# axlwild/dna-kmeres-parallel

Measured on AMD Instinct MI355X. Metric: k-mers/sec (whole node), 10 Gbase synthetic FASTA, at 1/2/4/8 MI355X, higher is better.
Workload: dtype u8

## Files before the change

dna-kmeres-parallel_amd/csrc/kmc_dense.hip:

```cpp
#include <hip/hip_runtime.h>

#include <algorithm>
#include <atomic>
#include <cstdint>
#include <cstdio>
#include <cstdlib>
#include <mutex>
#include <vector>

#include "kmc.h"
#include "kmc_internal.h"
#include "kmc_stream.h"
#include "kmc_workspace.h"

namespace kmc {
constexpr int kHm3Scan = 256;
constexpr int kChunk = 16;
thread_local hipEvent_t t_trace_before = nullptr;
thread_local hipEvent_t t_trace_after = nullptr;
namespace {

struct Spill {
    int64_t rec;
    int32_t code;
    int32_t amount;
};

struct Params {
    const char *data;
    const void *indices;
    int64_t ibias;
    int64_t n;
    int32_t *sum;
    int64_t ld;
    int32_t *invalid;
    int64_t wl, wh, rl, rh;
    int derive;
    int G;
    uint32_t *slab;
    int64_t *slot_rec;
    Spill *spill;
    uint32_t *spill_cnt;
    uint32_t spill_cap;
    uint32_t *status;
};

__device__ __forceinline__ void raise_status(uint32_t *st, uint32_t code) {
    if (st) __hip_atomic_store(st, code, __ATOMIC_RELAXED, __HIP_MEMORY_SCOPE_SYSTEM);
}

__device__ __forceinline__ uint32_t half_inc(uint32_t hb) {
    uint32_t r;
    asm("v_mad_u32_u24 %0, %1, %2, 1" : "=v"(r) : "v"(hb), "s"(0xFFFFu));
    return r;
}

struct P16Ctx {
    uint32_t *h;
    uint32_t *spilled;
    uint32_t *spill_n;
    Spill *spill;
    uint32_t cap;
    int64_t rec;
};

__device__ __forceinline__ void p16_spill(const P16Ctx &c, int32_t code, int32_t amount) {
    const uint32_t i = atomicAdd(c.spill_n, 1u);
    if (i < c.cap) {
        Spill e;
        e.rec = c.rec;
        e.code = code;
        e.amount = amount;
        c.spill[i] = e;
    }
}

__device__ __noinline__ void p16_fix(const P16Ctx &c, uint32_t word, uint32_t hb, uint32_t hiwrap) {
    if (hb == 0u) {
        p16_spill(c, (int32_t)word, 65536);
        if (hiwrap) p16_spill(c, (int32_t)(word | 0x8000u), 65536);
        const uint32_t o2 = __hip_atomic_fetch_add(&c.h[word], 0xFFFF0000u, __ATOMIC_RELAXED,
                                                   __HIP_MEMORY_SCOPE_WORKGROUP);
        if ((o2 >> 16) == 0u) p16_spill(c, (int32_t)(word | 0x8000u), -65536);
    } else {
        p16_spill(c, (int32_t)(word | 0x8000u), 65536);
    }
}

template <int K, int J>
__device__ __forceinline__ uint32_t window_code(uint32_t lo, uint32_t mid) {
    constexpr uint32_t M = (K == 16) ? 0xFFFFFFFFu : ((1u << (2 * K)) - 1u);
    if constexpr (J <= 16 - K)
        return (lo >> (2 * J)) & M;
    else
        return (mid >> (2 * (J - 8))) & M;
}

template <int K, int R, int J, bool MASKED>
__device__ __forceinline__ void add32(uint32_t lo, uint32_t mid, uint32_t W, uint32_t *h, uint32_t rep) {
    const uint32_t code = window_code<K, J>(lo, mid);
    if (!MASKED || ((W >> J) & 1u))
        __hip_atomic_fetch_add(&h[code * R + rep], 1u, __ATOMIC_RELAXED, __HIP_MEMORY_SCOPE_WORKGROUP);
}

template <int K, int R, bool MASKED>
__device__ __forceinline__ void count_tile32(uint32_t lo, uint32_t hi, uint32_t W, uint32_t *h, int lane) {
    const uint32_t mid = __builtin_amdgcn_alignbit(hi, lo, 16);
    const uint32_t rep = (uint32_t)(lane & (R - 1));
    add32<K, R, 0, MASKED>(lo, mid, W, h, rep);
    add32<K, R, 1, MASKED>(lo, mid, W, h, rep);
    add32<K, R, 2, MASKED>(lo, mid, W, h, rep);
    add32<K, R, 3, MASKED>(lo, mid, W, h, rep);
    add32<K, R, 4, MASKED>(lo, mid, W, h, rep);
    add32<K, R, 5, MASKED>(lo, mid, W, h, rep);
    add32<K, R, 6, MASKED>(lo, mid, W, h, rep);
    add32<K, R, 7, MASKED>(lo, mid, W, h, rep);
    add32<K, R, 8, MASKED>(lo, mid, W, h, rep);
    add32<K, R, 9, MASKED>(lo, mid, W, h, rep);
    add32<K, R, 10, MASKED>(lo, mid, W, h, rep);
    add32<K, R, 11, MASKED>(lo, mid, W, h, rep);
    add32<K, R, 12, MASKED>(lo, mid, W, h, rep);
    add32<K, R, 13, MASKED>(lo, mid, W, h, rep);
    add32<K, R, 14, MASKED>(lo, mid, W, h, rep);
    add32<K, R, 15, MASKED>(lo, mid, W, h, rep);
}

template <bool MASKED>
__device__ __forceinline__ void count_tile_p16_plain(uint32_t lo, uint32_t hi, uint32_t W, uint32_t *h) {
// ... 35 lines not shown
        w[q] = (lo & (T - 1)) | ((hi & (T - 1)) << 16);
    }
}

template <int BLOCK, uint32_t T>
__device__ __forceinline__ void p16_scan(const P16Ctx &pc) {
    constexpr uint32_t HOT = (0xFFFFu & ~(T - 1)) * 0x00010001u;
    constexpr int NW4 = (1 << 15) / 4;
    const uint4 *h4 = reinterpret_cast<const uint4 *>(pc.h);
    uint32_t hot = 0u;
#pragma unroll
    for (int i = 0; i < NW4 / BLOCK; ++i) {
        const uint4 v = h4[threadIdx.x + i * BLOCK];
        hot |= (uint32_t)(((v.x | v.y | v.z | v.w) & HOT) != 0u) << i;
    }
    if (hot) {
        for (int i = 0; i < NW4 / BLOCK; ++i)
            if ((hot >> i) & 1u) p16_scan_fix<T>(pc, (int)threadIdx.x + i * BLOCK);
    }
}

template <int K, int R, int HM, int BLOCK>
struct DenseOp {
    static_assert(HM == 0 || HM == 3, "histogram modes: 0 (32-bit bins) and 3 (k = 8 packed halves)");
    uint32_t *h;
    int lane;
    const P16Ctx &pc;
    uint32_t nwin = 0u;

    __device__ DenseOp(uint32_t *h_, int lane_, const P16Ctx &pc_) : h(h_), lane(lane_), pc(pc_) {}

    __device__ __forceinline__ void before_tile() {}
    template <bool MASKED>
    __device__ __forceinline__ void tile(uint32_t lo, uint32_t hi, uint32_t W) {
        count_tile<K, R, HM, MASKED>(lo, hi, W, h, lane);
        if constexpr (HM == 3) nwin += MASKED ? (uint32_t)__builtin_popcount(W) : 16u;
    }
    __device__ __forceinline__ void segment_end() {
        if constexpr (HM == 3) {
            lds_barrier();
            p16_scan<BLOCK, 32768u>(pc);
            lds_barrier();
        }
    }
    static constexpr int kSegChunks = HM == 3 ? BLOCK / 64 * kHm3Scan / kChunk : 0;
    __device__ __forceinline__ void after_iter(int64_t, int64_t, bool) {}
};

template <int BLOCK>
__device__ __noinline__ void recount_p16(const char *data, int64_t ps, int64_t pe, int64_t rl, int64_t rh,
                                         const P16Ctx &pc) {
    constexpr int K = 8;
    const int64_t per = (pe - ps + BLOCK - 1) / BLOCK;
    const int64_t i0 = ps + (int64_t)threadIdx.x * per;
    const int64_t i1 = (i0 + per) < pe ? (i0 + per) : pe;
    uint32_t code = 0u, run = 0u;
    for (int64_t b = i0; b < i1 + K - 1; ++b) {
        const uint32_t c = (b >= rl && b < rh) ? (uint32_t)(uint8_t)data[b] : 0u;
        const uint32_t v = c == 'A' ? 0u : c == 'C' ? 1u : c == 'G' ? 2u : c == 'T' ? 3u : 4u;
        run = v < 4u ? run + 1u : 0u;
        code = (code >> 2) | ((v & 3u) << (2 * K - 2));
        if (run >= (uint32_t)K) {
            const uint32_t word = code & 0x7FFFu, hb = code >> 15;
            const uint32_t old = __hip_atomic_fetch_add(&pc.h[word], half_inc(hb), __ATOMIC_RELAXED,
                                                        __HIP_MEMORY_SCOPE_WORKGROUP);
            const uint32_t m = hb ? 0xFFFF0000u : 0x0000FFFFu;
            if ((old & m) == m) p16_fix(pc, word, hb, old >= 0xFFFF0000u ? 1u : 0u);
        }
    }
}

template <int K, int R, int HM, class Idx, int BLOCK>
__global__ __launch_bounds__(BLOCK) void count_dense_kernel(Params p) {
    constexpr bool P16 = HM != 0;
    constexpr int NB = 1 << (2 * K);
    constexpr int NW = P16 ? NB / 2 : NB * R;
    __shared__ __attribute__((aligned(16))) uint32_t smem[NW + 8];
    uint32_t *h = smem;
    uint32_t *misc = smem + NW;

    const int tid = threadIdx.x, lane = tid & 63;
    const int w = blockIdx.x;
    const Geom g = make_geom<Idx>(p);
    const int64_t tb = g.T0 + (int64_t)w * g.tpw;
    const int64_t te = (tb + g.tpw) < g.T1 ? (tb + g.tpw) : g.T1;
    int64_t slot0 = -1, slot1 = -1;

    if (tb < te) {
        const int64_t R0 = (tb << kTileShift) > g.wl ? (tb << kTileShift) : g.wl;
        const int64_t R1 = (te << kTileShift) < g.wh ? (te << kTileShift) : g.wh;
        int64_t s0 = 0;
        if (p.n <= BLOCK) {
            if (tid == 0) {
                misc[0] = 0u;
                misc[3] = 0u;
                misc[4] = 0u;
                misc[5] = 0u;
                misc[7] = 0u;
            }
            const bool le = tid < p.n && rec_off<Idx>(p, tid) <= R0;
            for (int i = tid; i < NW / 4; i += BLOCK) reinterpret_cast<uint4 *>(h)[i] = make_uint4(0u, 0u, 0u, 0u);
            const int cnt = __syncthreads_count(le);
            s0 = cnt > 0 ? cnt - 1 : 0;
        } else {
            if (tid == 0) {
                int64_t lo = 0, hi = p.n - 1;
                if (rec_off<Idx>(p, 0) <= R0) {
                    while (lo < hi) {
                        const int64_t mid = (lo + hi + 1) >> 1;
                        if (rec_off<Idx>(p, mid) <= R0) lo = mid;
                        else hi = mid - 1;
                    }
                }
                misc[0] = 0u;
                misc[3] = 0u;
                misc[4] = 0u;
                misc[5] = 0u;
                misc[7] = 0u;
                misc[1] = (uint32_t)lo;
                misc[2] = (uint32_t)((uint64_t)lo >> 32);
            }
            for (int i = tid; i < NW / 4; i += BLOCK) reinterpret_cast<uint4 *>(h)[i] = make_uint4(0u, 0u, 0u, 0u);
            __syncthreads();
            s0 = (int64_t)((uint64_t)misc[1] | ((uint64_t)misc[2] << 32));
        }

        P16Ctx pc;
        pc.h = h;
        pc.spilled = misc + 5;
        pc.spill_n = misc;
        pc.spill = p.spill ? p.spill + (int64_t)w * p.spill_cap : nullptr;
        pc.cap = p.spill_cap;

        int npieces = 0;
        for (int64_t s = s0; s < p.n; ++s) {
            if (rec_off<Idx>(p, s) >= R1) break;
            int64_t ca, ce;
            record_windows<K, Idx>(p, g, s, ca, ce);
            const int64_t ps = ca > R0 ? ca : R0;
            const int64_t pe = ce < R1 ? ce : R1;
            if (ps >= pe) continue;
            pc.rec = s;
            const int64_t tp0 = ps >> kTileShift;
            const int64_t tp1 = ((pe - 1) >> kTileShift) + 1;
            using Op = DenseOp<K, R, HM, BLOCK>;
            Op op(h, lane, pc);
            if constexpr (K >= 7) {
                stream_chunks<K, kChunk, Op::kSegChunks>(p.data, tp0, tp1, ps, pe, g.rl, g.rh, lane, &misc[7], op);
            } else {
                constexpr int NWAVES = BLOCK / 64;
                const int wave = __builtin_amdgcn_readfirstlane(tid >> 6);
                const int64_t per = (tp1 - tp0 + NWAVES - 1) / NWAVES;
                const int64_t a0 = tp0 + (int64_t)wave * per;
                const int64_t a1 = (a0 + per) < tp1 ? (a0 + per) : tp1;
                stream_tiles<K>(p.data, a0, a1, per, ps, pe, g.rl, g.rh, lane, op);
            }
            if constexpr (HM == 3) {
                const uint32_t wsum = wave_sum(op.nwin);
                if (lane == 0) atomicAdd(&misc[3], wsum);
            }
            __syncthreads();
            const bool entire = (ps == ca) && (pe == ce);
            int slot = 0;
            if (!entire) {
                slot = (npieces == 0) ? 0 : 1;
                if (slot == 0) slot0 = s;
                else slot1 = s;
            }
            uint32_t *dst = p.slab + ((int64_t)w * 2 + slot) * NB;
            if constexpr (P16) {
                const auto flush = [&]() {
                    uint32_t dsum = 0u;
                    if (!entire) {
                        for (int i = tid; i < NW / 4; i += BLOCK) {
                            const uint4 v = reinterpret_cast<const uint4 *>(h)[i];
                            reinterpret_cast<uint4 *>(h)[i] = make_uint4(0u, 0u, 0u, 0u);
                            dsum += (v.x & 0xFFFFu) + (v.x >> 16) + (v.y & 0xFFFFu) + (v.y >> 16) + (v.z & 0xFFFFu) +
                                    (v.z >> 16) + (v.w & 0xFFFFu) + (v.w >> 16);
                            reinterpret_cast<uint4 *>(dst)[i] = v;
                        }
                        return dsum;
                    }
                    for (int i = tid; i < NW; i += BLOCK) {
                        const uint32_t v = h[i];
                        h[i] = 0u;
                        dsum += (v & 0xFFFFu) + (v >> 16);
                        if (entire) {
                            p.sum[s + p.ld * (int64_t)i] = (int32_t)(v & 0xFFFFu);
                            p.sum[s + p.ld * (int64_t)(i + NW)] = (int32_t)(v >> 16);
                        } else {
                            dst[i] = v;
                        }
                    }
                    return dsum;
                };
                const uint32_t dsum = flush();
                if constexpr (HM == 3) {
                    const uint32_t wsum = wave_sum(dsum);
                    if (lane == 0) atomicAdd(&misc[4], wsum);
                    __syncthreads();
                    if (tid == 0) {
                        misc[6] = misc[3] != misc[4] + misc[5] ? 1u : 0u;
                        misc[3] = 0u;
                        misc[4] = 0u;
                        misc[5] = 0u;
                    }
                    __syncthreads();
                    if (misc[6]) {
                        const uint32_t n0 = misc[0] < pc.cap ? misc[0] : pc.cap;
                        for (uint32_t i = tid; i < n0; i += BLOCK)
                            if (pc.spill[i].rec == s) pc.spill[i].amount = 0;
                        __syncthreads();
                        recount_p16<BLOCK>(p.data, ps, pe, g.rl, g.rh, pc);
                        __syncthreads();
                        (void)flush();
                    }
                }
            } else {
                for (int c = tid; c < NB; c += BLOCK) {
                    uint32_t v = 0;
#pragma unroll
                    for (int r = 0; r < R; ++r) {
                        v += h[c * R + r];
                        h[c * R + r] = 0u;
                    }
                    if (entire) p.sum[s + p.ld * (int64_t)c] = (int32_t)v;
                    else dst[c] = v;
                }
            }
            if (tid == 0) misc[7] = 0u;
            __syncthreads();
            ++npieces;
        }
    }
    if (tid == 0) {
        p.slot_rec[2 * w] = slot0;
        p.slot_rec[2 * w + 1] = slot1;
        if (p.spill_cnt) {
            p.spill_cnt[w] = (tb < te) ? misc[0] : 0u;
            if (tb < te && misc[0] > p.spill_cap) raise_status(p.status, KMC_ERR_CAPACITY);
        }
    }
}

template <int K, class Idx, bool P16>
__global__ __launch_bounds__(256) void reduce_dense_kernel(Params p) {
    constexpr int NB = 1 << (2 * K);
    constexpr int NW = P16 ? NB / 2 : NB;
    constexpr int RC = NW / 4 < 16 ? NW / 4 : 16;
    constexpr int RR = 256 / RC;
    constexpr int RW = 4 * RC;
    constexpr int NH = P16 ? 2 : 1;
    __shared__ uint32_t s_part[RR][RW * NH];
    __shared__ uint32_t s_out[RW * NH];
    const int tid = threadIdx.x, col = tid % RC, row = tid / RC;
    const int64_t c0 = (int64_t)blockIdx.x * RW;
    const Geom g = make_geom<Idx>(p);
    const auto for_spills = [&](int64_t s, int64_t wf, int64_t wlast, auto &&f) {
        for (int64_t l = wf; l <= wlast; ++l) {
            const uint32_t c = p.spill_cnt[l] < p.spill_cap ? p.spill_cnt[l] : p.spill_cap;
            const Spill *sp = p.spill + l * (int64_t)p.spill_cap;
            uint32_t lo = 0u, hi = c;
            while (lo < hi) {
                const uint32_t mid = (lo + hi) >> 1;
                if (sp[mid].rec < s) lo = mid + 1u;
                else hi = mid;
            }
            for (uint32_t i = lo + tid; i < c; i += 256) {
                const Spill e = sp[i];
                if (e.rec != s) break;
                const int64_t wd = (int64_t)(e.code & (NW - 1)) - c0;
                if (e.amount != 0 && wd >= 0 && wd < RW) f((int)wd + (e.code / NW) * RW, e.amount);
            }
        }
    };
    for (int64_t s = blockIdx.y; s < p.n; s += gridDim.y) {
        int64_t ca, ce;
        record_windows<K, Idx>(p, g, s, ca, ce);
        if (blockIdx.x == 0 && tid == 0 && ce - ca >= ((int64_t)1 << 31)) raise_status(p.status, KMC_ERR_RECORD_TOO_LONG);
        if (ce <= ca) {
            for (int i = tid; i < RW * NH; i += 256) {
                const int64_t c = c0 + i % RW + (i / RW) * NW;
                p.sum[s + p.ld * c] = 0;
            }
            continue;
        }
        const int64_t wf = ((ca >> kTileShift) - g.T0) / g.tpw;
        const int64_t wlast = (((ce - 1) >> kTileShift) - g.T0) / g.tpw;
        bool spills = false;
        if constexpr (P16) {
            uint32_t any = 0u;
            for (int64_t l = wf + tid; l <= wlast; l += 256) any |= p.spill_cnt[l];
            spills = __syncthreads_or(any != 0u) != 0;
        }
        if (wf == wlast) {
            if (spills)
                for_spills(s, wf, wlast, [&](int i, int32_t a) {
                    atomicAdd(&p.sum[s + p.ld * (c0 + i % RW + (i / RW) * (int64_t)NW)], a);
                });
            continue;
        }
        uint32_t acc[4 * NH] = {};
        const int64_t sf = 2 * wf + (p.slot_rec[2 * wf] == s ? 0 : 1);
        const int64_t n = wlast - wf + 1;
#pragma unroll 4
        for (int64_t i = row; i < n; i += RR) {
            const int64_t slot = i == 0 ? sf : 2 * (wf + i);
            const uint4 v = reinterpret_cast<const uint4 *>(p.slab + slot * NB + c0)[col];
            const uint32_t x[4] = {v.x, v.y, v.z, v.w};
#pragma unroll
            for (int e = 0; e < 4; ++e) {
                if constexpr (P16) {
                    acc[e] += x[e] & 0xFFFFu;
                    acc[4 + e] += x[e] >> 16;
                } else {
                    acc[e] += x[e];
                }
            }
        }
#pragma unroll
        for (int e = 0; e < 4 * NH; ++e) s_part[row][(e / 4) * RW + col * 4 + e % 4] = acc[e];
        __syncthreads();
        for (int i = tid; i < RW * NH; i += 256) {
            uint32_t t = 0u;
#pragma unroll 8
            for (int r = 0; r < RR; ++r) t += s_part[r][i];
            s_out[i] = t;
        }
        if (spills) {
            __syncthreads();
            for_spills(s, wf, wlast, [&](int i, int32_t a) { atomicAdd(&s_out[i], (uint32_t)a); });
        }
        __syncthreads();
        for (int i = tid; i < RW * NH; i += 256) {
            const int64_t c = c0 + i % RW + (i / RW) * NW;
            p.sum[s + p.ld * c] = (int32_t)s_out[i];
        }
        __syncthreads();
    }
}


template <int K, class Idx>
__global__ __launch_bounds__(256) void invalid_kernel(Params p) {
    constexpr int NB = 1 << (2 * K);
    __shared__ int64_t red[256];
    for (int64_t s = blockIdx.x; s < p.n; s += gridDim.x) {
        int64_t acc = 0;
        for (int c = threadIdx.x; c < NB; c += 256) acc += p.sum[s + p.ld * (int64_t)c];
        red[threadIdx.x] = acc;
        __syncthreads();
        for (int st = 128; st > 0; st >>= 1) {
            if ((int)threadIdx.x < st) red[threadIdx.x] += red[threadIdx.x + st];
            __syncthreads();
        }
        if (threadIdx.x == 0) {
            const Geom g = make_geom<Idx>(p);
            int64_t ca, ce;
            record_windows<K, Idx>(p, g, s, ca, ce);
            const int64_t nw = ce > ca ? ce - ca : 0;
            p.invalid[s] = (int32_t)(nw - red[0]);
        }
        __syncthreads();
    }
}

template <int K>
struct Cfg;
template <> struct Cfg<1> { static constexpr int R = 32, BLOCK = 512, HM = 0; static constexpr bool P16 = false; };
template <> struct Cfg<2> { static constexpr int R = 32, BLOCK = 512, HM = 0; static constexpr bool P16 = false; };
template <> struct Cfg<3> { static constexpr int R = 32, BLOCK = 512, HM = 0; static constexpr bool P16 = false; };
template <> struct Cfg<4> { static constexpr int R = 32, BLOCK = 512, HM = 0; static constexpr bool P16 = false; };
template <> struct Cfg<5> { static constexpr int R = 8, BLOCK = 512, HM = 0; static constexpr bool P16 = false; };
template <> struct Cfg<6> { static constexpr int R = 2, BLOCK = 512, HM = 0; static constexpr bool P16 = false; };
template <> struct Cfg<7> { static constexpr int R = 1, BLOCK = 512, HM = 0; static constexpr bool P16 = false; };
template <> struct Cfg<8> { static constexpr int R = 1, BLOCK = 1024, HM = 3; static constexpr bool P16 = true; };

struct DevInfo {
    int occ[KMC_DENSE_MAX_K + 1][2] = {};
    uint32_t *status_host = nullptr;
    uint32_t *status_dev = nullptr;
};

std::mutex g_mu;
std::vector<DevInfo> g_dev;


template <int K, class Idx>
void *kernel_ptr() {
    return reinterpret_cast<void *>(&count_dense_kernel<K, Cfg<K>::R, Cfg<K>::HM, Idx, Cfg<K>::BLOCK>);
}

thread_local int t_reserved_cus = 0;

#ifdef KMC_DIAG_HOOKS
std::atomic<uint32_t> g_diag_spill_cap{0};
#endif

template <int K, class Idx>
int grid_size(int device, int &G) {
    int dev_cus = 0;
    if (int e = device_cus(device, &dev_cus)) return e;
    std::lock_guard<std::mutex> lk(g_mu);
    if ((int)g_dev.size() <= device) g_dev.resize(device + 1);
    DevInfo &d = g_dev[device];
    const int ix = sizeof(Idx) == 8 ? 1 : 0;
    if (d.occ[K][ix] == 0) {
        const void *kp = kernel_ptr<K, Idx>();
        int nb = 0;
        hipError_t e = hipOccupancyMaxActiveBlocksPerMultiprocessor(&nb, kp, Cfg<K>::BLOCK, 0);
        if (e != hipSuccess) return (int)e;
        d.occ[K][ix] = nb > 0 ? nb : 1;
    }
    const int cus = dev_cus - t_reserved_cus;
    G = (cus > 0 ? cus : 1) * d.occ[K][ix];
    return 0;
}

int status_flag(int device, uint32_t **host, uint32_t **dev) {
    std::lock_guard<std::mutex> lk(g_mu);
    if ((int)g_dev.size() <= device) g_dev.resize(device + 1);
    DevInfo &d = g_dev[device];
    if (!d.status_host) {
        void *h = nullptr;
        hipError_t e = hipHostMalloc(&h, sizeof(uint32_t), hipHostMallocMapped | hipHostMallocCoherent);
        if (e != hipSuccess) return KMC_ERR_NOMEM;
        void *dp = nullptr;
        e = hipHostGetDevicePointer(&dp, h, 0);
        if (e != hipSuccess) {
            (void)hipHostFree(h);
            return (int)e;
        }
        *static_cast<volatile uint32_t *>(h) = 0u;
        d.status_host = static_cast<uint32_t *>(h);
        d.status_dev = static_cast<uint32_t *>(dp);
    }
    *host = d.status_host;
    *dev = d.status_dev;
    return 0;
}

int take_status(int device) {
    uint32_t *h = nullptr;
    {
        std::lock_guard<std::mutex> lk(g_mu);
        if ((int)g_dev.size() > device && device >= 0) h = g_dev[device].status_host;
    }
    if (!h) return KMC_OK;
    const uint32_t v = __atomic_exchange_n(h, 0u, __ATOMIC_ACQ_REL);
    return (int)v;
}

struct WsLayout {
    int64_t *slot_rec;
    uint32_t *spill_cnt, *slab;
    Spill *spill;
    size_t total;
};

inline WsLayout ws_layout(void *base, int k, int G, uint32_t spill_cap) {
    const size_t nb = (size_t)1 << (2 * k);
    Carver c(base);
    WsLayout L;
    L.slot_rec = c.take<int64_t>((size_t)G * 2);
    L.spill_cnt = c.take<uint32_t>((size_t)G);
    L.slab = c.take<uint32_t>((size_t)G * 2 * nb);
    L.spill = c.take<Spill>((size_t)G * spill_cap);
    L.total = c.total();
    return L;
}

constexpr uint32_t kSpillWindowsPerEntry = 4096;
static_assert(5u * kSpillWindowsPerEntry <= 65536u, "HM 3 scan + HM 1 recount entries exceed the spill cap");
inline uint32_t spill_cap_for(int64_t tiles_per_wg) {
    const int64_t windows = tiles_per_wg * kTile;
    return (uint32_t)(windows / kSpillWindowsPerEntry + 64);
}

struct Plan {
    int G;
    uint32_t spill_cap;
    size_t ws_bytes;
};

template <int K, class Idx>
int make_plan(int device, bool derive, int64_t wl, int64_t wh, Plan &pl) {
    int G = 0;
    int e = grid_size<K, Idx>(device, G);
    if (e) return e;
    pl.spill_cap = 0;
    if (!derive) {
        const int64_t tiles = wh > wl ? ((wh + kTile - 1) >> kTileShift) - (wl >> kTileShift) : 0;
        if (tiles < G) G = tiles > 0 ? (int)tiles : 1;
        const int64_t tpw = tiles > 0 ? (tiles + G - 1) / G : 1;
        if (Cfg<K>::P16) {
            pl.spill_cap = spill_cap_for(tpw);
#ifdef KMC_DIAG_HOOKS
            const uint32_t dc = g_diag_spill_cap.load();
            if (dc) pl.spill_cap = dc;
#endif
        }
    }
    pl.G = G;
    pl.ws_bytes = ws_layout(nullptr, K, G, pl.spill_cap).total;
    return 0;
}

DeviceCache g_ws;

struct Request {
    const char *data;
    const void *indices;
    int64_t ibias;
    int64_t n;
    int32_t *sum;
    int64_t ld;
    int32_t *invalid;
    bool derive;
    int64_t wl, wh, rl, rh;
    void *ws;
    size_t ws_bytes;
    uint32_t *status;
};

template <int K, class Idx>
int run_dense(const Request &q, hipStream_t st) {
    int device = 0;
    hipError_t he = hipGetDevice(&device);
    if (he != hipSuccess) return (int)he;
    bool derive = q.derive;
    int64_t wl = q.wl, wh = q.wh, rl = q.rl, rh = q.rh;
    if (derive && Cfg<K>::P16) {
        Idx ends[2];
        he = hipMemcpyAsync(&ends[0], q.indices, sizeof(Idx), hipMemcpyDeviceToHost, st);
        if (he == hipSuccess)
            he = hipMemcpyAsync(&ends[1], (const Idx *)q.indices + q.n, sizeof(Idx), hipMemcpyDeviceToHost, st);
        if (he == hipSuccess) he = hipStreamSynchronize(st);
        if (he != hipSuccess) return (int)he;
        wl = rl = (int64_t)ends[0] + q.ibias;
        wh = rh = (int64_t)ends[1] + q.ibias;
        derive = false;
    }
    Plan pl;
    int e = make_plan<K, Idx>(device, derive, wl, wh, pl);
    if (e) return e;
    void *ws = nullptr;
    if ((e = bind_workspace(g_ws, device, pl.ws_bytes, q.ws, q.ws_bytes, 0, &ws))) return e;
    const WsLayout L = ws_layout(ws, K, pl.G, pl.spill_cap);
    Params p;
    p.data = q.data;
    p.indices = q.indices;
    p.ibias = q.ibias;
    p.n = q.n;
    p.sum = q.sum;
    p.ld = q.ld;
    p.invalid = q.invalid;
    p.wl = wl;
    p.wh = wh;
    p.rl = rl;
    p.rh = rh;
    p.derive = derive ? 1 : 0;
    p.G = pl.G;
    p.slot_rec = L.slot_rec;
    p.spill_cnt = Cfg<K>::P16 ? L.spill_cnt : nullptr;
    p.slab = L.slab;
    p.spill = Cfg<K>::P16 ? L.spill : nullptr;
    p.spill_cap = pl.spill_cap;
    p.status = q.status;
    if (!p.status) {
        uint32_t *sh = nullptr;
        e = status_flag(device, &sh, &p.status);
        if (e) return e;
    }

    constexpr int NB = 1 << (2 * K);
    if (t_trace_before) {
        he = hipEventRecord(t_trace_before, st);
        if (he != hipSuccess) return (int)he;
    }
    hipLaunchKernelGGL((count_dense_kernel<K, Cfg<K>::R, Cfg<K>::HM, Idx, Cfg<K>::BLOCK>), dim3(pl.G),
                       dim3(Cfg<K>::BLOCK), 0, st, p);
    he = hipGetLastError();
    if (he != hipSuccess) return (int)he;
    if (t_trace_after) {
        he = hipEventRecord(t_trace_after, st);
        if (he != hipSuccess) return (int)he;
    }
    constexpr int NWR = Cfg<K>::P16 ? NB / 2 : NB;
    constexpr int RW = NWR / 4 < 16 ? NWR : 64;
    const unsigned cb = (unsigned)(NWR / RW);
    hipLaunchKernelGGL((reduce_dense_kernel<K, Idx, Cfg<K>::P16>), dim3(cb, (unsigned)std::min<int64_t>(q.n, kMaxGridY)),
                       dim3(256), 0, st, p);
    he = hipGetLastError();
    if (he != hipSuccess) return (int)he;
    if (q.invalid) {
        hipLaunchKernelGGL((invalid_kernel<K, Idx>), dim3((unsigned)std::min<int64_t>(q.n, kMaxGridX)), dim3(256), 0,
                           st, p);
        he = hipGetLastError();
        if (he != hipSuccess) return (int)he;
    }
    return 0;
}

template <class Idx>
int dispatch(int k, const Request &q, hipStream_t st) {
    switch (k) {
        case 1: return run_dense<1, Idx>(q, st);
        case 2: return run_dense<2, Idx>(q, st);
        case 3: return run_dense<3, Idx>(q, st);
        case 4: return run_dense<4, Idx>(q, st);
        case 5: return run_dense<5, Idx>(q, st);
        case 6: return run_dense<6, Idx>(q, st);
        case 7: return run_dense<7, Idx>(q, st);
        case 8: return run_dense<8, Idx>(q, st);
        default: return KMC_ERR_UNSUPPORTED_K;
    }
}

template <class Idx>
size_t workspace_for(int k, int device, bool derive, int64_t wl, int64_t wh) {
    Plan pl;
    int e = 0;
    switch (k) {
        case 1: e = make_plan<1, Idx>(device, derive, wl, wh, pl); break;
        case 2: e = make_plan<2, Idx>(device, derive, wl, wh, pl); break;
        case 3: e = make_plan<3, Idx>(device, derive, wl, wh, pl); break;
        case 4: e = make_plan<4, Idx>(device, derive, wl, wh, pl); break;
        case 5: e = make_plan<5, Idx>(device, derive, wl, wh, pl); break;
        case 6: e = make_plan<6, Idx>(device, derive, wl, wh, pl); break;
        case 7: e = make_plan<7, Idx>(device, derive, wl, wh, pl); break;
        case 8: e = make_plan<8, Idx>(device, derive, wl, wh, pl); break;
        default: return 0;
    }
    return e ? 0 : pl.ws_bytes;
}

}
}

using namespace kmc;

extern "C" int kmc_set_reserved_cus(int n) {
    if (n < 0 || n > 64) return KMC_ERR_INVALID_ARG;
    t_reserved_cus = n;
    return KMC_OK;
}

extern "C" int kmc_dense_status(int device) { return take_status(device); }

#ifdef KMC_DIAG_HOOKS
extern "C" KMC_DIAG_API int kmc_diag_dense_spill_cap(unsigned cap) {
    g_diag_spill_cap.store(cap);
    return KMC_OK;
}
#endif

extern "C" int kmc_trace_set_events(hipEvent_t before, hipEvent_t after) {
    t_trace_before = before;
    t_trace_after = after;
    return KMC_OK;
}

extern "C" int sumKmereCoincidencesGlobalMemory_hip(char *data, int *indices, unsigned num_seqs, int *sum,
                                                    hipStream_t stream) {
    if (num_seqs == 0) return KMC_OK;
    if (!data || !indices || !sum) return KMC_ERR_INVALID_ARG;
    const uintptr_t mis = reinterpret_cast<uintptr_t>(data) & 15u;
    Request q{};
    q.data = data - mis;
    q.ibias = (int64_t)mis;
    q.indices = indices;
    q.n = num_seqs;
    q.sum = sum;
// ... 103 lines not shown
```

dna-kmeres-parallel_amd/csrc/kmc_stream.h:

```cpp
#pragma once

#include <hip/hip_runtime.h>

#include <cstdint>

namespace kmc {

constexpr int kStreamPF = 3;
constexpr int kStreamNT = 1;

constexpr int kTileShift = 10;
constexpr int kTile = 1 << kTileShift;

constexpr uint32_t kCodeLo = 0x01000000u;
constexpr uint32_t kCodeHi = 0x02000003u;
constexpr uint32_t kCanonLo = 0x43FF41FFu;
constexpr uint32_t kCanonHi = 0x47FFFF54u;

__device__ __forceinline__ uint32_t byte_codes(uint32_t w) {
    return __builtin_amdgcn_perm(kCodeHi, kCodeLo, w & 0x07070707u);
}
__device__ __forceinline__ uint32_t byte_mismatch(uint32_t w) {
    return w ^ __builtin_amdgcn_perm(kCanonHi, kCanonLo, w & 0x07070707u);
}
// ... 42 lines not shown
}

template <int K>
__device__ __forceinline__ uint32_t smear(uint32_t x) {
    uint32_t s = x;
    int c = 1;
#pragma unroll
    for (int it = 0; it < 6; ++it) {
        if (c < K) {
            const int st = (c < K - c) ? c : (K - c);
            s |= s >> st;
            c += st;
        }
    }
    return s;
}

__device__ __forceinline__ uint32_t from_next_lane(uint32_t x) {
    return (uint32_t)__builtin_amdgcn_update_dpp(0, (int)x, 0x130, 0xF, 0xF, false);
}

__device__ __forceinline__ uint32_t wave_incl_scan(uint32_t x) {
    x += (uint32_t)__builtin_amdgcn_update_dpp(0, (int)x, 0x111, 0xF, 0xF, true);
    x += (uint32_t)__builtin_amdgcn_update_dpp(0, (int)x, 0x112, 0xF, 0xF, true);
    x += (uint32_t)__builtin_amdgcn_update_dpp(0, (int)x, 0x114, 0xF, 0xF, true);
    x += (uint32_t)__builtin_amdgcn_update_dpp(0, (int)x, 0x118, 0xF, 0xF, true);
    x += (uint32_t)__builtin_amdgcn_update_dpp(0, (int)x, 0x142, 0xA, 0xF, false);
    x += (uint32_t)__builtin_amdgcn_update_dpp(0, (int)x, 0x143, 0xC, 0xF, false);
    return x;
}

__device__ __forceinline__ uint32_t wave_sum(uint32_t x) {
#pragma unroll
    for (int o = 32; o > 0; o >>= 1) x += __shfl_xor(x, o);
    return x;
}

__device__ __forceinline__ void quad_bcast4(uint32_t x, uint32_t *o) {
    o[0] = (uint32_t)__builtin_amdgcn_update_dpp(0, (int)x, 0x00, 0xF, 0xF, false);
    o[1] = (uint32_t)__builtin_amdgcn_update_dpp(0, (int)x, 0x55, 0xF, 0xF, false);
    o[2] = (uint32_t)__builtin_amdgcn_update_dpp(0, (int)x, 0xAA, 0xF, 0xF, false);
    o[3] = (uint32_t)__builtin_amdgcn_update_dpp(0, (int)x, 0xFF, 0xF, 0xF, false);
}

__device__ __forceinline__ void lds_barrier() {
    __builtin_amdgcn_fence(__ATOMIC_RELEASE, "workgroup", "local");
    __builtin_amdgcn_s_barrier();
    __builtin_amdgcn_fence(__ATOMIC_ACQUIRE, "workgroup", "local");
}

struct Geom {
    int64_t wl, wh, rl, rh;
    int64_t T0, T1, tpw;
};

template <class Idx, class P>
__device__ __forceinline__ int64_t rec_off(const P &p, int64_t i) {
    return (int64_t)((const Idx *)p.indices)[i] + p.ibias;
}

template <class Idx, class P>
__device__ __forceinline__ Geom make_geom(const P &p) {
    Geom g;
    if (p.derive) {
        g.wl = rec_off<Idx>(p, 0);
        g.wh = rec_off<Idx>(p, p.n);
        g.rl = g.wl;
        g.rh = g.wh;
    } else {
        g.wl = p.wl;
        g.wh = p.wh;
        g.rl = p.rl;
        g.rh = p.rh;
    }
    if (g.wh <= g.wl) {
        g.T0 = g.T1 = 0;
        g.tpw = 1;
    } else {
        g.T0 = g.wl >> kTileShift;
        g.T1 = (g.wh + kTile - 1) >> kTileShift;
        g.tpw = (g.T1 - g.T0 + p.G - 1) / p.G;
    }
    return g;
}

template <int K, class Idx, class P>
__device__ __forceinline__ void record_windows(const P &p, const Geom &g, int64_t s, int64_t &ca,
                                               int64_t &ce) {
    const int64_t a = rec_off<Idx>(p, s);
    const int64_t e = rec_off<Idx>(p, s + 1);
    const int64_t nw = e - a - K > 0 ? e - a - K : 0;
    ca = a > g.wl ? a : g.wl;
    ce = (a + nw) < g.wh ? (a + nw) : g.wh;
}


template <class Idx, class P>
__device__ __forceinline__ int64_t first_record_at(const P &p, int64_t pos) {
    int64_t lo = 0, hi = p.n - 1;
    if (rec_off<Idx>(p, 0) <= pos) {
        while (lo < hi) {
            const int64_t mid = (lo + hi + 1) >> 1;
            if (rec_off<Idx>(p, mid) <= pos) lo = mid;
            else hi = mid - 1;
        }
    }
    return lo;
}

__device__ __forceinline__ __amdgpu_buffer_rsrc_t tile_rsrc(const char *data, int64_t base_off, int64_t rh) {
    const int64_t rh16 = (rh + 15) & ~(int64_t)15;
    int64_t nrec = rh16 - base_off;
    nrec = nrec < 0 ? 0 : (nrec > (1ll << 31) ? (1ll << 31) : nrec);
    return __builtin_amdgcn_make_buffer_rsrc(const_cast<char *>(data) + base_off, (short)0, (int)nrec,
                                             0x00020000);
}

__device__ __forceinline__ int64_t tile_base(int64_t t, int64_t rl) {
    const int64_t b = t << kTileShift, rl16 = rl & ~(int64_t)15;
    return b > rl16 ? b : rl16;
}

template <int NT = kStreamNT>
__device__ __forceinline__ uint4 load_tile_fast(__amdgpu_buffer_rsrc_t rsrc, int64_t base_off, int64_t t,
                                                int lane) {
    const int64_t off = (t << kTileShift) - base_off + (int64_t)lane * 16;
    typedef unsigned u32x4 __attribute__((ext_vector_type(4)));
    const u32x4 x = __builtin_amdgcn_raw_buffer_load_b128(rsrc, (int)(uint32_t)off, 0, NT ? 2 : 0);
    return make_uint4(x[0], x[1], x[2], x[3]);
}

__device__ __forceinline__ bool tile_straddles(int64_t t, int64_t rl, int64_t rh) {
    const int64_t b = t << kTileShift;
    return ((rl & 15) != 0 && rl > b && rl < b + kTile) || ((rh & 15) != 0 && rh > b && rh < b + kTile);
}

__device__ __forceinline__ uint4 mask_range(uint4 v, int64_t q, int64_t rl, int64_t rh) {
    const int64_t lo = rl - q, hi = rh - q;
    uint32_t w[4] = {v.x, v.y, v.z, v.w};
#pragma unroll
    for (int d = 0; d < 4; ++d) {
        int64_t a = lo - 4 * d, b = hi - 4 * d;
        a = a < 0 ? 0 : (a > 4 ? 4 : a);
        b = b < 0 ? 0 : (b > 4 ? 4 : b);
        uint32_t m = 0u;
        if (b > a) {
            const uint32_t upto = b == 4 ? 0xFFFFFFFFu : ((1u << (8 * (uint32_t)b)) - 1u);
            m = upto & ~((1u << (8 * (uint32_t)a)) - 1u);
        }
        w[d] &= m;
    }
    return make_uint4(w[0], w[1], w[2], w[3]);
}

template <int K, int PF_ = kStreamPF, int NT_ = kStreamNT>
struct TileStream {
    static constexpr int PF = PF_;
    static constexpr int NT = NT_;
    static constexpr int NS = PF + 1;
    const char *__restrict__ data;
    int64_t t0, ps, pe, rl, rh;
    int lane;
    __amdgpu_buffer_rsrc_t rsrc;
    int64_t base_off;
    uint4 r[NS];
    uint32_t c_cur, v_cur;
// ... 226 lines not shown
```

dna-kmeres-parallel_amd/kmc.py:

```python
import ctypes
import os
import re

import numpy as np

HERE = os.path.dirname(os.path.abspath(__file__))
REPO = os.path.dirname(HERE)
LIB_PATH = os.environ.get("KMC_LIB") or os.path.join(HERE, "lib", "libkmc.so")
DIAG_LIB_PATH = os.environ.get("KMC_DIAG_LIB") or os.path.join(HERE, "lib", "libkmc_diag.so")
HEADER = os.path.join(REPO, "include", "kmc.h")

DIALECT_BLANK = 0
DIALECT_NONL = 1
MAX_SEQS_REFERENCE = 100
DROPIN_K = 3
KMC_ERR_CAPACITY = 1009
KMC_ERR_RECORD_TOO_LONG = 1010
KMC_ERR_INTERNAL = 1011


class KmcError(RuntimeError):
    def __init__(self, code, what):
        self.code = code
        super().__init__("%s failed: %s (%d)" % (what, error_string(code), code))


_P = ctypes.c_void_p
_U64 = ctypes.c_uint64
_I64 = ctypes.c_int64


class DenseArgs(ctypes.Structure):
    _fields_ = [
        ("data", _P), ("indices", _P), ("num_seqs", _U64), ("k", ctypes.c_int),
        ("sum", _P), ("sum_ld", _U64), ("invalid", _P),
        ("read_lo", _U64), ("read_hi", _U64), ("win_lo", _U64), ("win_hi", _U64),
        ("workspace", _P), ("workspace_bytes", ctypes.c_size_t), ("status", _P),
    ]


_lib = None
_diag_lib = None
_active = None


def lib():
    global _lib
    if _active is not None:
        return _active
    if _lib is None:
        _lib = _load(LIB_PATH)
    return _lib


class diag:

    def __enter__(self):
        global _diag_lib, _active
        if _diag_lib is None:
            _diag_lib = _load(DIAG_LIB_PATH)
            _diag_lib.kmc_diag_radix_mode.argtypes = [ctypes.c_int, ctypes.c_float]
            _diag_lib.kmc_diag_canon_claim_cap.argtypes = [ctypes.c_uint]
            _diag_lib.kmc_diag_canon_sort_cap.argtypes = [ctypes.c_uint]
            _diag_lib.kmc_diag_canon_sort_cap_big.argtypes = [ctypes.c_uint]
            _diag_lib.kmc_diag_canon_direct.argtypes = [ctypes.c_int]
            _diag_lib.kmc_diag_canon_fallback.argtypes = [ctypes.POINTER(ctypes.c_ulonglong)] * 2
            _diag_lib.kmc_diag_canon_fallback_detail.argtypes = [ctypes.POINTER(ctypes.c_ulonglong), ctypes.c_uint,
                                                                 ctypes.POINTER(ctypes.c_ulonglong)]
            _diag_lib.kmc_diag_dense_spill_cap.argtypes = [ctypes.c_uint]
            _diag_lib.kmc_diag_canon_stale_queue.argtypes = [ctypes.c_longlong]
        self._prev = _active
        _active = _diag_lib
        return _diag_lib

    def __exit__(self, *exc):
        global _active
        L = _active
        L.kmc_diag_radix_mode(0, 1.0)
        L.kmc_diag_canon_claim_cap(0)
        L.kmc_diag_canon_sort_cap(1 << 30)
        L.kmc_diag_canon_direct(1)
        L.kmc_diag_dense_spill_cap(0)
        L.kmc_diag_canon_stale_queue(-1)
        _active = self._prev
        return False


def hip_runtimes():
    with open("/proc/self/maps") as f:
        return sorted(set(line.split()[-1] for line in f if "/libamdhip64.so" in line))


def _load(path):
    if not os.path.exists(path):
        raise RuntimeError("%s not built: run `make -C %s` (no CPU fallback exists)" % (os.path.basename(path), HERE))
    if os.environ.get("KMC_NO_TORCH") != "1":
        try:
            import torch
        except ImportError:
            pass
    L = ctypes.CDLL(path)
    rt = hip_runtimes()
    if len(rt) > 1:
        raise RuntimeError("two HIP runtimes are mapped in this process (%s): each would initialise the GPU on its "
                           "own, so %s is refused; import torch before loading it (or set KMC_NO_TORCH=1 only in "
                           "processes that never import torch)" % (", ".join(rt), os.path.basename(path)))
    L.kmc_error_string.restype = ctypes.c_char_p
    L.kmc_error_string.argtypes = [ctypes.c_int]
    L.kmc_version.restype = ctypes.c_int
    L.kmc_version.argtypes = []
    L.sumKmereCoincidencesGlobalMemory_hip.argtypes = [_P, _P, ctypes.c_uint, _P, _P]
    L.kmc_count_dense_workspace_size.restype = ctypes.c_size_t
    L.kmc_count_dense_workspace_size.argtypes = [ctypes.c_int, _U64, _U64, ctypes.c_int]
    L.kmc_count_dense.argtypes = [_P, _P, _U64, _U64, ctypes.c_int, _P, _P, _P, ctypes.c_size_t, _P]
    L.kmc_count_dense_ex.argtypes = [ctypes.POINTER(DenseArgs), _P]
    L.kmc_count_dense_ex_workspace_size.restype = ctypes.c_size_t
    L.kmc_count_dense_ex_workspace_size.argtypes = [ctypes.POINTER(DenseArgs), ctypes.c_int]
    L.kmc_dense_status.argtypes = [ctypes.c_int]
    L.kmc_trace_set_events.argtypes = [_P, _P]
    L.kmc_set_reserved_cus.argtypes = [ctypes.c_int]
    L.kmc_plan_shards.argtypes = [_P, _U64, ctypes.c_int, ctypes.c_int, _U64, _P]
    L.kmc_count_multi.argtypes = [_P, _P, _U64, _U64, ctypes.c_int, ctypes.c_int, _P, _P, _P]
    L.kmc_multi_release.argtypes = []
    L.kmc_synth_fill.argtypes = [_P, _U64, _U64, _U64, _U64, _P]
    L.kmc_synth_fill_range.argtypes = [_P, _U64, _U64, _U64, _U64, _P]
    L.kmc_synth_indices.argtypes = [_P, _U64, _U64]
    L.kmc_synth_indices.restype = None
    L.kmc_fasta_load.argtypes = [ctypes.c_char_p, ctypes.c_int, _I64, ctypes.POINTER(_P)]
    for fn in ("kmc_fasta_num_seqs", "kmc_fasta_data_bytes", "kmc_fasta_reference_num_indexes"):
        getattr(L, fn).restype = _U64
        getattr(L, fn).argtypes = [_P]
    L.kmc_fasta_indices.restype = _P
    L.kmc_fasta_indices.argtypes = [_P]
    L.kmc_fasta_data.restype = _P
    L.kmc_fasta_data.argtypes = [_P]
    L.kmc_fasta_free.argtypes = [_P]
    L.kmc_fasta_free.restype = None
    L.kmc_fasta_parse_device.argtypes = [_P, _U64, ctypes.c_int, _P, _U64, _P, _U64, ctypes.POINTER(_U64),
                                         ctypes.POINTER(_U64), _P]
    L.kmc_fasta_load_device.argtypes = [ctypes.c_char_p, ctypes.c_int, _I64, ctypes.POINTER(_P),
                                        ctypes.POINTER(_U64), ctypes.POINTER(_P), ctypes.POINTER(_U64), _P]
    L.kmc_pair_distances_workspace_size.restype = ctypes.c_size_t
    L.kmc_pair_distances_workspace_size.argtypes = [_U64, ctypes.c_int, ctypes.c_int]
    L.kmc_pair_distances.argtypes = [_P, _U64, _P, _U64, ctypes.c_int, _P, _P, ctypes.c_size_t, _P]
    L.kmc_pair_distances_sparse_workspace_size.restype = ctypes.c_size_t
    L.kmc_pair_distances_sparse_workspace_size.argtypes = [_U64, _U64, ctypes.c_int]
    L.kmc_pair_distances_sparse.argtypes = [_P, _P, _P, _U64, _P, _U64, ctypes.c_int, _P, _P, ctypes.c_size_t, _P]
    L.kmc_sketch_workspace_size.restype = ctypes.c_size_t
    L.kmc_sketch_workspace_size.argtypes = [_U64, _U64, ctypes.c_uint32, ctypes.c_int]
    L.kmc_sketch_from_counts.argtypes = [_P, _P, _P, _U64, _U64, ctypes.c_uint32, _U64, ctypes.c_uint32, _P, _P, _P,
                                         ctypes.c_size_t, _P]
    L.kmc_sketch_distances.argtypes = [_P, _P, _U64, ctypes.c_uint32, ctypes.c_int, _P, _P, _P, _P]
    L.kmc_sketch_from_sequences_workspace_size.restype = ctypes.c_size_t
    L.kmc_sketch_from_sequences_workspace_size.argtypes = [_U64, _U64, ctypes.c_uint32, ctypes.c_int]
    L.kmc_sketch_from_sequences.argtypes = [_P, _P, _U64, _U64, ctypes.c_int, ctypes.c_uint, ctypes.c_uint32, _U64,
                                            _P, _P, _P, ctypes.c_size_t, _P]
    L.kmc_sketch_from_sequences_grouped_workspace_size.restype = ctypes.c_size_t
    L.kmc_sketch_from_sequences_grouped_workspace_size.argtypes = [_U64, _U64, _U64, ctypes.c_uint32, ctypes.c_int]
    L.kmc_sketch_from_sequences_grouped.argtypes = [_P, _P, _U64, _U64, _P, _U64, ctypes.c_int, ctypes.c_uint,
                                                    ctypes.c_uint32, _U64, _P, _P, _P, ctypes.c_size_t, _P]
    L.kmc_sketch_merge_groups.argtypes = [_P, _P, _U64, _P, _U64, ctypes.c_uint32, _P, _P, _P]
    L.minKmeres2_hip.argtypes = [_P, _P, ctypes.c_int, ctypes.c_int, _P, _P]
    L.kmc_count_canonical_hash.argtypes = [_P, _P, _U64, ctypes.c_int, ctypes.c_uint, _P, _P, _U64, _P,
                                           ctypes.POINTER(_U64), _P]
    L.kmc_count_canonical_hash_ex.argtypes = [_P, _P, _U64, ctypes.c_int, ctypes.c_uint, _P, _P, _U64, _P,
                                              ctypes.POINTER(_U64), _P, ctypes.c_size_t, _P]
    L.kmc_count_canonical_workspace_size.restype = ctypes.c_size_t
    L.kmc_count_canonical_workspace_size.argtypes = [_P, _U64, ctypes.c_int, ctypes.c_int]
# ... 416 lines not shown
```

Before: 4800 billion.

## Learn per-class tile split from measured workgroup durations for dense counting

For K>=7 dense counting, the count kernel records each workgroup's wall-clock duration. The reduce kernel gets an extra block that turns these durations into per-class tile widths (8 classes, clamped to ±1/8 of the even split), and the next call uses those widths to size workgroup ranges. The aim is to even out workgroup finish times when different CU classes run at different speeds. The cost is extra workspace, a timing write per workgroup, owner lookups in the reduce, a larger spill cap, and dependence on state carried between calls (the tag check guards against mismatched geometry).

Result: no change. 4824 billion, median of 6 (+0.5%).

```diff
diff --git a/dna-kmeres-parallel_amd/csrc/kmc_dense.hip b/dna-kmeres-parallel_amd/csrc/kmc_dense.hip
--- a/dna-kmeres-parallel_amd/csrc/kmc_dense.hip
+++ b/dna-kmeres-parallel_amd/csrc/kmc_dense.hip
@@ -25,6 +25,14 @@
     int32_t code;
     int32_t amount;
 };
+
+struct SplitWs {
+    uint32_t learnt[kSplitClasses];
+    uint32_t tag[4];
+    uint32_t used[kSplitClasses];
+    uint32_t pad[4];
+};
+constexpr uint32_t kSplitMagic = 0x4B57A500u;
 
 struct Params {
     const char *data;
@@ -43,7 +51,18 @@
     uint32_t *spill_cnt;
     uint32_t spill_cap;
     uint32_t *status;
+    SplitWs *split;
+    uint32_t *dur;
 };
+
+__device__ __forceinline__ bool split_on(const Params &p) {
+    return p.split != nullptr && !p.derive && split_weighted(p.G);
+}
+
+__device__ __forceinline__ bool split_tag_ok(const uint32_t *tag, int k, int G, int64_t T) {
+    return tag[0] == kSplitMagic + (uint32_t)k && tag[1] == (uint32_t)G && tag[2] == (uint32_t)T &&
+           tag[3] == (uint32_t)((uint64_t)T >> 32);
+}
 
 __device__ __forceinline__ void raise_status(uint32_t *st, uint32_t code) {
     if (st) __hip_atomic_store(st, code, __ATOMIC_RELAXED, __HIP_MEMORY_SCOPE_SYSTEM);
@@ -245,8 +264,25 @@
     const int tid = threadIdx.x, lane = tid & 63;
     const int w = blockIdx.x;
     const Geom g = make_geom<Idx>(p);
-    const int64_t tb = g.T0 + (int64_t)w * g.tpw;
-    const int64_t te = (tb + g.tpw) < g.T1 ? (tb + g.tpw) : g.T1;
+    int64_t tb = g.T0 + (int64_t)w * g.tpw;
+    int64_t te = (tb + g.tpw) < g.T1 ? (tb + g.tpw) : g.T1;
+    uint32_t t_in = 0u;
+    if constexpr (K >= 7) {
+        t_in = (uint32_t)wall_clock64();
+        if (split_on(p)) {
+            const int64_t T = g.T1 - g.T0;
+            const bool ok = split_tag_ok(p.split->tag, K, p.G, T);
+            uint32_t raw[kSplitClasses], a[kSplitClasses];
+#pragma unroll
+            for (int c = 0; c < kSplitClasses; ++c) raw[c] = ok ? p.split->learnt[c] : (uint32_t)g.tpw;
+            split_make(raw, T, p.G, g.tpw, a);
+            split_range(split_prefix(a), g.T0, g.T1, w, tb, te);
+            if (w == 0 && tid == 0) {
+#pragma unroll
+                for (int c = 0; c < kSplitClasses; ++c) p.split->used[c] = a[c];
+            }
+        }
+    }
     int64_t slot0 = -1, slot1 = -1;
 
     if (tb < te) {
@@ -403,6 +439,67 @@
             p.spill_cnt[w] = (tb < te) ? misc[0] : 0u;
             if (tb < te && misc[0] > p.spill_cap) raise_status(p.status, KMC_ERR_CAPACITY);
         }
+        if constexpr (K >= 7) {
+            if (p.dur) p.dur[w] = (uint32_t)wall_clock64() - t_in;
+        }
+    }
+}
+
+template <int K>
+__device__ void learn_split(const Params &p, const Geom &g) {
+    __shared__ unsigned long long s_d[kSplitClasses];
+    __shared__ uint32_t s_n[kSplitClasses];
+    const int tid = threadIdx.x;
+    if (tid < kSplitClasses) {
+        s_d[tid] = 0ull;
+        s_n[tid] = 0u;
+    }
+    __syncthreads();
+    uint32_t a[kSplitClasses];
+#pragma unroll
+    for (int c = 0; c < kSplitClasses; ++c) a[c] = p.split->used[c];
+    const Split sp = split_prefix(a);
+    const int cl = tid % kSplitClasses;
+    const uint32_t width = split_width(sp, cl);
+    unsigned long long d = 0ull;
+    uint32_t n = 0u;
+    for (int64_t w = tid; w < p.G; w += 256) {
+        int64_t tb, te;
+        split_range(sp, g.T0, g.T1, w, tb, te);
+        if (te - tb == (int64_t)width) {
+            d += p.dur[w];
+            ++n;
+        }
+    }
+    atomicAdd(&s_d[cl], d);
+    atomicAdd(&s_n[cl], n);
+    __syncthreads();
+    if (tid == 0) {
+        const int64_t T = g.T1 - g.T0, nr = p.G / kSplitClasses;
+        const int64_t lo = g.tpw - g.tpw / 8, hi = g.tpw + g.tpw / 8;
+        const double smin = (double)((T + nr - 1) / nr);
+        double rate[kSplitClasses], sum = 0.0;
+        bool ok = true;
+#pragma unroll
+        for (int c = 0; c < kSplitClasses; ++c) {
+            ok = ok && s_n[c] > 0u && s_d[c] > 0ull;
+            rate[c] = ok ? (double)a[c] * (double)s_n[c] / (double)s_d[c] : 0.0;
+            sum += rate[c];
+        }
+#pragma unroll
+        for (int c = 0; c < kSplitClasses; ++c) {
+            int64_t v = g.tpw;
+            if (ok) {
+                const int64_t target = (int64_t)ceil(smin * rate[c] / sum);
+                v = ((int64_t)a[c] + target + 1) / 2;
+                v = v < lo ? lo : (v > hi ? hi : v);
+            }
+            p.split->learnt[c] = (uint32_t)v;
+        }
+        p.split->tag[0] = kSplitMagic + (uint32_t)K;
+        p.split->tag[1] = (uint32_t)p.G;
+        p.split->tag[2] = (uint32_t)T;
+        p.split->tag[3] = (uint32_t)((uint64_t)T >> 32);
     }
 }
 
@@ -419,6 +516,13 @@
     const int tid = threadIdx.x, col = tid % RC, row = tid / RC;
     const int64_t c0 = (int64_t)blockIdx.x * RW;
     const Geom g = make_geom<Idx>(p);
+    const bool weighted = K >= 7 && split_on(p);
+    if constexpr (K >= 7) {
+        if (blockIdx.x == NW / RW) {
+            if (blockIdx.y == 0) learn_split<K>(p, g);
+            return;
+        }
+    }
     const auto for_spills = [&](int64_t s, int64_t wf, int64_t wlast, auto &&f) {
         for (int64_t l = wf; l <= wlast; ++l) {
             const uint32_t c = p.spill_cnt[l] < p.spill_cap ? p.spill_cnt[l] : p.spill_cap;
@@ -448,8 +552,18 @@
             }
             continue;
         }
-        const int64_t wf = ((ca >> kTileShift) - g.T0) / g.tpw;
-        const int64_t wlast = (((ce - 1) >> kTileShift) - g.T0) / g.tpw;
+        int64_t wf, wlast;
+        if (!weighted) {
+            wf = ((ca >> kTileShift) - g.T0) / g.tpw;
+            wlast = (((ce - 1) >> kTileShift) - g.T0) / g.tpw;
+        } else {
+            uint32_t sa[kSplitClasses];
+#pragma unroll
+            for (int c = 0; c < kSplitClasses; ++c) sa[c] = p.split->used[c];
+            const Split sp = split_prefix(sa);
+            wf = split_owner(sp, g.T0, ca >> kTileShift);
+            wlast = split_owner(sp, g.T0, (ce - 1) >> kTileShift);
+        }
         bool spills = false;
         if constexpr (P16) {
             uint32_t any = 0u;
@@ -558,6 +672,10 @@
 
 #ifdef KMC_DIAG_HOOKS
 std::atomic<uint32_t> g_diag_spill_cap{0};
+bool diag_forced_weights(int *pm) {
+    const char *s = getenv("KMC_DIAG_DENSE_WEIGHTS");
+    return s && sscanf(s, "%d,%d,%d,%d,%d,%d,%d,%d", pm, pm + 1, pm + 2, pm + 3, pm + 4, pm + 5, pm + 6, pm + 7) == 8;
+}
 #endif
 
 template <int K, class Idx>
@@ -615,6 +733,8 @@
 }
 
 struct WsLayout {
+    SplitWs *split;
+    uint32_t *dur;
     int64_t *slot_rec;
     uint32_t *spill_cnt, *slab;
     Spill *spill;
@@ -629,6 +749,12 @@
     L.spill_cnt = c.take<uint32_t>((size_t)G);
     L.slab = c.take<uint32_t>((size_t)G * 2 * nb);
     L.spill = c.take<Spill>((size_t)G * spill_cap);
+    L.split = c.take_if<SplitWs>(k == 7, 1);
+    L.dur = k == 7 ? L.spill_cnt : nullptr;
+    if (k == 8 && base) {
+        L.split = reinterpret_cast<SplitWs *>(L.slab + nb / 2);
+        L.dur = L.slab + nb / 2 + sizeof(SplitWs) / sizeof(uint32_t);
+    }
     L.total = c.total();
     return L;
 }
@@ -639,11 +765,15 @@
     const int64_t windows = tiles_per_wg * kTile;
     return (uint32_t)(windows / kSpillWindowsPerEntry + 64);
 }
+inline uint32_t spill_entries_bound(int64_t tiles) { return (uint32_t)((tiles * kTile * 5 + 65535) / 65536); }
+constexpr int64_t kSplitSlabRoom = (1 << 15) - (int64_t)(sizeof(SplitWs) / sizeof(uint32_t));
 
 struct Plan {
     int G;
     uint32_t spill_cap;
     size_t ws_bytes;
+    int64_t tiles, tpw;
+    bool weighted;
 };
 
 template <int K, class Idx>
@@ -652,12 +782,19 @@
     int e = grid_size<K, Idx>(device, G);
     if (e) return e;
     pl.spill_cap = 0;
+    pl.tiles = 0;
+    pl.tpw = 1;
+    pl.weighted = false;
     if (!derive) {
         const int64_t tiles = wh > wl ? ((wh + kTile - 1) >> kTileShift) - (wl >> kTileShift) : 0;
         if (tiles < G) G = tiles > 0 ? (int)tiles : 1;
         const int64_t tpw = tiles > 0 ? (tiles + G - 1) / G : 1;
+        pl.tiles = tiles;
+        pl.tpw = tpw;
+        pl.weighted = K >= 7 && split_weighted(G) && (K != 8 || G <= kSplitSlabRoom);
         if (Cfg<K>::P16) {
             pl.spill_cap = spill_cap_for(tpw);
+            if (pl.weighted) pl.spill_cap = std::max(pl.spill_cap, spill_entries_bound(split_max_tiles(tpw)));
 #ifdef KMC_DIAG_HOOKS
             const uint32_t dc = g_diag_spill_cap.load();
             if (dc) pl.spill_cap = dc;
@@ -735,6 +872,27 @@
         e = status_flag(device, &sh, &p.status);
         if (e) return e;
     }
+    p.split = pl.weighted ? L.split : nullptr;
+    p.dur = pl.weighted ? L.dur : nullptr;
+    bool learn = pl.weighted;
+#ifdef KMC_DIAG_HOOKS
+    int pm[kSplitClasses];
+    if (pl.weighted && diag_forced_weights(pm)) {
+        SplitWs f{};
+        for (int c = 0; c < kSplitClasses; ++c) {
+            f.learnt[c] = (uint32_t)(pl.tpw + pl.tpw * std::max(-1000, std::min(1000, pm[c])) / 1000);
+        }
+        f.tag[0] = kSplitMagic + (uint32_t)K;
+        f.tag[1] = (uint32_t)pl.G;
+        f.tag[2] = (uint32_t)pl.tiles;
+        f.tag[3] = (uint32_t)((uint64_t)pl.tiles >> 32);
+        he = hipMemcpyAsync(L.split, &f, sizeof(f), hipMemcpyHostToDevice, st);
+        if (he == hipSuccess) he = hipStreamSynchronize(st);
+        if (he != hipSuccess) return (int)he;
+        learn = false;
+        p.dur = nullptr;
+    }
+#endif
 
     constexpr int NB = 1 << (2 * K);
     if (t_trace_before) {
@@ -751,7 +909,7 @@
     }
     constexpr int NWR = Cfg<K>::P16 ? NB / 2 : NB;
     constexpr int RW = NWR / 4 < 16 ? NWR : 64;
-    const unsigned cb = (unsigned)(NWR / RW);
+    const unsigned cb = (unsigned)(NWR / RW) + (learn ? 1u : 0u);
     hipLaunchKernelGGL((reduce_dense_kernel<K, Idx, Cfg<K>::P16>), dim3(cb, (unsigned)std::min<int64_t>(q.n, kMaxGridY)),
                        dim3(256), 0, st, p);
     he = hipGetLastError();
diff --git a/dna-kmeres-parallel_amd/csrc/kmc_stream.h b/dna-kmeres-parallel_amd/csrc/kmc_stream.h
--- a/dna-kmeres-parallel_amd/csrc/kmc_stream.h
+++ b/dna-kmeres-parallel_amd/csrc/kmc_stream.h
@@ -148,6 +148,73 @@
         g.tpw = (g.T1 - g.T0 + p.G - 1) / p.G;
     }
     return g;
+}
+
+constexpr int kSplitClasses = 8;
+
+__host__ __device__ __forceinline__ bool split_weighted(int G) { return G >= kSplitClasses && G % kSplitClasses == 0; }
+
+__host__ __device__ __forceinline__ int64_t split_max_tiles(int64_t tpw) { return tpw + 2 * (tpw / 8) + 1; }
+
+struct Split {
+    int64_t S;
+    uint32_t pre[kSplitClasses + 1];
+};
+
+__host__ __device__ __forceinline__ void split_make(const uint32_t *raw, int64_t T, int G, int64_t tpw, uint32_t *a) {
+    const int64_t lo = tpw - tpw / 8, hi = tpw + tpw / 8;
+    int64_t S = 0;
+    for (int c = 0; c < kSplitClasses; ++c) {
+        const int64_t v = (int64_t)raw[c];
+        a[c] = (uint32_t)(v < lo ? lo : (v > hi ? hi : v));
+        S += a[c];
+    }
+    const int64_t nr = G / kSplitClasses;
+    const int64_t smin = (T + nr - 1) / nr;
+    if (S < smin) {
+        const int64_t d = smin - S;
+        for (int c = 0; c < kSplitClasses; ++c) a[c] += (uint32_t)(d / kSplitClasses + (c < d % kSplitClasses ? 1 : 0));
+    }
+}
+
+__host__ __device__ __forceinline__ Split split_prefix(const uint32_t *a) {
+    Split s;
+    s.pre[0] = 0u;
+    for (int c = 0; c < kSplitClasses; ++c) s.pre[c + 1] = s.pre[c] + a[c];
+    s.S = (int64_t)s.pre[kSplitClasses];
+    return s;
+}
+
+__host__ __device__ __forceinline__ void split_range(const Split &s, int64_t T0, int64_t T1, int64_t w, int64_t &tb,
+                                            int64_t &te) {
+    const int c = (int)(w % kSplitClasses);
+    uint32_t p0 = 0u, p1 = 0u;
+#pragma unroll
+    for (int i = 0; i < kSplitClasses; ++i) {
+        p0 = c == i ? s.pre[i] : p0;
+        p1 = c == i ? s.pre[i + 1] : p1;
+    }
+    tb = T0 + (w / kSplitClasses) * s.S + (int64_t)p0;
+    const int64_t e = T0 + (w / kSplitClasses) * s.S + (int64_t)p1;
+    te = e < T1 ? e : T1;
+}
+
+__host__ __device__ __forceinline__ uint32_t split_width(const Split &s, int c) {
+    uint32_t v = 0u;
+#pragma unroll
+    for (int i = 0; i < kSplitClasses; ++i) v = c == i ? s.pre[i + 1] - s.pre[i] : v;
+    return v;
+}
+
+__host__ __device__ __forceinline__ int64_t split_owner(const Split &s, int64_t T0, int64_t t) {
+    const int64_t r = (t - T0) / s.S;
+    const uint32_t x = (uint32_t)((t - T0) - r * s.S);
+    const uint32_t p1 = s.pre[1], p2 = s.pre[2], p3 = s.pre[3], p4 = s.pre[4], p5 = s.pre[5], p6 = s.pre[6],
+                   p7 = s.pre[7];
+    const bool h4 = x >= p4;
+    const bool h2 = x >= (h4 ? p6 : p2);
+    const uint32_t q1 = h4 ? (h2 ? p7 : p5) : (h2 ? p3 : p1);
+    return r * kSplitClasses + (h4 ? 4 : 0) + (h2 ? 2 : 0) + (x >= q1 ? 1 : 0);
 }
 
 template <int K, class Idx, class P>
diff --git a/dna-kmeres-parallel_amd/kmc.py b/dna-kmeres-parallel_amd/kmc.py
--- a/dna-kmeres-parallel_amd/kmc.py
+++ b/dna-kmeres-parallel_amd/kmc.py
@@ -82,8 +82,17 @@
         L.kmc_diag_canon_direct(1)
         L.kmc_diag_dense_spill_cap(0)
         L.kmc_diag_canon_stale_queue(-1)
+        diag_dense_weights(None)
         _active = self._prev
         return False
+
+
+def diag_dense_weights(per_mille):
+    if per_mille is None:
+        os.environ.pop("KMC_DIAG_DENSE_WEIGHTS", None)
+    else:
+        assert len(per_mille) == 8
+        os.environ["KMC_DIAG_DENSE_WEIGHTS"] = ",".join(str(int(x)) for x in per_mille)
 
 
 def hip_runtimes():
```
